# SinOncology/BreakID

Measured on AMD Instinct MI355X. Metric: M reads/s clustered+split-scanned, higher is better.
Workload: dtype int32/u8 (+f64 sd replay)

## Files before the change

### breakid_amd/csrc/sortemu.h

```cpp
#pragma once
#include "bk_common.h"
#include "prims.h"
#include <vector>
#include <atomic>

struct SortService
{
  DevBuf ctl, slots[2], seq[2], jobs, dbg, pos[2];
  uint32_t pos_cap[2] = {0, 0};
  uint32_t cap[2] = {0, 0};
  hipStream_t st[2] = {nullptr, nullptr}, quit_stream = nullptr, st_copy = nullptr;
  uint32_t *quit_host = nullptr;
  uint32_t *quit_dev = nullptr;
  uint32_t cap32 = 0;
  uint32_t quit_word = 0, starts = 0;
  size_t wide_lds = 0;
  bool running = false;
  std::atomic<uint32_t> next_slot{0};
  uint32_t stats[8] = {};
  void start(uint64_t n_bound, uint64_t max_group, hipStream_t after);
  bool narrow_running(double seconds) const;
  void stop();
  uint32_t new_slot() { return next_slot.fetch_add(1u); }
  ~SortService();
  SortService() = default;
  SortService(const SortService &) = delete;
  SortService &operator=(const SortService &) = delete;
};

struct SortEmuBufs
{
  SortService *svc = nullptr;
  uint32_t svc_slot = 0xFFFFFFFFu, svc_epoch = 0;
  DevBuf cnt, err, segs_a, segs_b, posL, posR, scan_tmp, heap_list, heap_scratch, scratch32, scratch32b, fin_list, lv_tile, lv_segbase, lv_tileseg, lv_bar, chk_key0, chk_cnt, chk_bad, rk_a, rk_b, heap_tickets;
  prims::RadixBufs radix;
  std::vector<uint32_t> *heavy = nullptr;
  bool heavy_all = false;
  bool fork_heaps = true;
  DevBuf tj_ctl, tj_jobs, tj_slots[2], tj_seq[2], tj_pos[2], tj_heavy, tj_trace;
  uint32_t tj_cap[2] = {0, 0}, tj_epoch = 0;
  bool tj_ready = false;
  uint64_t sorts[3] = {0, 0, 0};
  static constexpr int N_AUX = 5;
  hipStream_t aux[N_AUX] = {};
  hipEvent_t fork = nullptr, join[N_AUX] = {};
  SortEmuBufs() = default;
  SortEmuBufs(const SortEmuBufs &) = delete;
  SortEmuBufs &operator=(const SortEmuBufs &) = delete;
  ~SortEmuBufs()
  {
    for (int i = 0; i < N_AUX; ++i)
    {
      if (aux[i]) (void) hipStreamDestroy(aux[i]);
      if (join[i]) (void) hipEventDestroy(join[i]);
    }
    if (fork) (void) hipEventDestroy(fork);
  }
};

bool sort_tasks_on();

void std_sort_groups(uint32_t *key, uint32_t *idx, const uint32_t *gof, const uint64_t *goff, uint32_t ng, uint64_t n, SortEmuBufs &b, hipStream_t st);
```

### breakid_amd/csrc/sortemu.hip

```cpp
#include "bk_common.h"
#include "prims.h"
#include "sortemu.h"
#include <vector>
#include <mutex>
#include <algorithm>
#include <cstdio>
#include <chrono>
#include <thread>
#include <cstdlib>
#include <ctime>

namespace
{
inline double now_ms()
{
  timespec ts;
  clock_gettime(CLOCK_MONOTONIC, &ts);
  return ts.tv_sec * 1e3 + ts.tv_nsec * 1e-6;
}
typedef __attribute__((address_space(1))) uint32_t gu32_t;
__device__ __forceinline__ void st_through(uint32_t *p, uint32_t v) { __hip_atomic_store((gu32_t *) p, v, __ATOMIC_RELAXED, __HIP_MEMORY_SCOPE_AGENT); }
struct Seg
{
  uint32_t first, last;
  uint32_t pivot;
  int32_t depth;
  uint32_t cut;
  uint32_t cbase;
};

constexpr uint32_t FIN_MAX = 2048;
constexpr uint32_t HEAP_BIG_MIN = 4096;
constexpr uint32_t LV_TILE = 2048;
__device__ __forceinline__ void lv_mark_tiles(uint32_t *__restrict__ tile_seg, uint32_t s, uint32_t cbase, uint32_t size)
{
// ... 2230 lines not shown
__global__ __launch_bounds__(256) void k_chk_keys(const uint32_t *__restrict__ key, const uint32_t *__restrict__ idx, const uint32_t *__restrict__ key0, uint32_t n, uint32_t *__restrict__ bad)
{
  const uint32_t p = blockIdx.x * blockDim.x + threadIdx.x;
  if (p >= n) return;
  const uint32_t x = idx[p];
  if (x < n && key0[x] != key[p])
  {
    atomicAdd(&bad[4], 1u);
    atomicMin(&bad[5], p);
  }
}
static void sort_check(const char *phase, const uint32_t *key, const uint32_t *idx, const uint32_t *key0, uint32_t n, const uint64_t *goff, uint32_t ng, hipStream_t st, SortEmuBufs &b)
{
  uint32_t *c = b.chk_cnt.as<uint32_t>(n), *bd = b.chk_bad.as<uint32_t>(8);
  const uint32_t init[8] = {0, 0, 0xFFFFFFFFu, 0xFFFFFFFFu, 0, 0xFFFFFFFFu, 0, 0};
  HIP_CHECK(hipDeviceSynchronize());
  HIP_CHECK(hipMemset(c, 0, (size_t) n * 4));
  HIP_CHECK(hipMemcpy(bd, init, 32, hipMemcpyHostToDevice));
  hipLaunchKernelGGL(k_chk_count, dim3(cdiv(n, 256)), dim3(256), 0, st, idx, n, c, bd);
  hipLaunchKernelGGL(k_chk_keys, dim3(cdiv(n, 256)), dim3(256), 0, st, key, idx, key0, n, bd);
  uint32_t h[8];
  HIP_CHECK(hipMemcpyAsync(h, bd, 32, hipMemcpyDeviceToHost, st));
  HIP_CHECK(hipStreamSynchronize(st));
  if (h[0] || h[1] || h[4])
  {
    std::vector<uint64_t> go((size_t) ng + 1);
    HIP_CHECK(hipMemcpy(go.data(), goff, ((size_t) ng + 1) * 8, hipMemcpyDeviceToHost));
    auto grp = [&](uint32_t p) { return p == 0xFFFFFFFFu ? -1 : (int) (std::upper_bound(go.begin(), go.end(), (uint64_t) p) - go.begin()) - 1; };
    fprintf(stderr, "[sortemu] CHECK FAILED %s: %u payloads out of range (first at %u), %u duplicated payloads (first at position %u, group %d), %u elements whose key is not their own (first at %u, group %d); n=%u\n",
            phase, h[0], h[2], h[1], h[3], grp(h[3]), h[4], h[5], grp(h[5]), n);
  }
}

static SvcParams svc_params(SortService &S)
{
  SvcParams P;
  uint32_t *ctl = S.ctl.get<uint32_t>();
  for (int k = 0; k < 2; ++k)
  {
    P.q[k].head = ctl + 64 * k;
    P.q[k].tail = ctl + 64 * k + 32;
    P.q[k].slots = S.slots[k].get<SvcTask>();
    P.q[k].seq = S.seq[k].get<uint32_t>();
    P.q[k].mask = S.cap[k] - 1;
    P.q[k].release = 1u;
  }
  P.error = ctl + 128;
  P.stats = ctl + 160;
  P.jobs = S.jobs.get<SvcJob>();
  P.quit_d = ctl + 192;
  P.host = S.quit_dev;
  P.cap32 = S.cap32;
  P.quit_word = S.quit_word;
  P.dbg = S.dbg.get<uint32_t>();
  for (int k = 0; k < 2; ++k)
  {
    P.pos[k] = S.pos[k].get<uint32_t>();
    P.pos_cap[k] = S.pos_cap[k];
  }
  P.timeout_ticks = SVC_TIMEOUT_TICKS;
  return P;
}
void SortService::start(uint64_t n_bound, uint64_t max_group, hipStream_t after)
{
  if (running) return;
  quit_stream = after;
  int dev = 0, cus = 0;
  HIP_CHECK(hipGetDevice(&dev));
  HIP_CHECK(hipDeviceGetAttribute(&cus, hipDeviceAttributeMultiprocessorCount, dev));
  const int n_wide = std::min(1024, std::max(4, cus / 4));
  const int n_narrow = std::max(8, 2 * (cus - n_wide));
  if (!quit_host)
  {
    HIP_CHECK(hipHostMalloc(reinterpret_cast<void **>(&quit_host), SVC_H_WORDS * 4, hipHostMallocMapped));
    HIP_CHECK(hipHostGetDevicePointer(reinterpret_cast<void **>(&quit_dev), quit_host, 0));
    for (int k = 0; k < 2; ++k) HIP_CHECK(hipStreamCreateWithFlags(&st[k], hipStreamNonBlocking));
    HIP_CHECK(hipStreamCreateWithFlags(&st_copy, hipStreamNonBlocking));
    hipFuncAttributes fa;
    HIP_CHECK(hipFuncGetAttributes(&fa, reinterpret_cast<const void *>(k_sort_service<true>)));
    wide_lds = (size_t) ((160u * 1024u - (uint32_t) fa.sharedSizeBytes) & ~15u);
    cap32 = (uint32_t) (wide_lds / 4 - 3);
    if ((cap32 & 1u) == 0) --cap32;
    HIP_CHECK(hipFuncSetAttribute(reinterpret_cast<const void *>(k_sort_service<true>), hipFuncAttributeMaxDynamicSharedMemorySize, (int) wide_lds));
    HIP_CHECK(hipFuncSetAttribute(reinterpret_cast<const void *>(k_sort_service<false>), hipFuncAttributeMaxDynamicSharedMemorySize, (int) SVC_NARROW_LDS));
  }
  auto pow2 = [](uint64_t v) {
    uint32_t c = 1024;
    while (c < v && c < (1u << 30)) c <<= 1;
    return c;
  };
  cap[0] = pow2(n_bound / HEAP_BIG_MIN + 4096);
  cap[1] = pow2(n_bound / 16 + 4096);
  (void) ctl.as<uint32_t>(256);
  for (int k = 0; k < 2; ++k)
  {
    (void) slots[k].as<SvcTask>(cap[k]);
    (void) seq[k].as<uint32_t>(cap[k]);
  }
  (void) jobs.as<SvcJob>(SVC_MAX_JOBS);
  pos_cap[0] = (uint32_t) std::max<uint64_t>(max_group, SVC_WIDE_MIN) + 64;
  pos_cap[1] = SVC_WIDE_MIN + 64;
  (void) pos[0].as<uint32_t>(2ull * pos_cap[0] * (uint64_t) n_wide);
  (void) pos[1].as<uint32_t>(2ull * pos_cap[1] * (uint64_t) n_narrow);
  if (bk_debug("svc"))
  {
    (void) dbg.as<uint32_t>(12 * 8192 + 48);
    HIP_CHECK(hipMemsetAsync(dbg.p, 0, (12 * 8192 + 48) * 4, after));
  }
  __atomic_store_n(quit_host, 0u, __ATOMIC_SEQ_CST);
  quit_word = 0xC0DE0000u | (++starts & 0xFFFFu);
  for (uint32_t k = 1; k < SVC_H_WORDS; ++k) quit_host[k] = 0u;
  next_slot = 0;
  const SvcParams P = svc_params(*this);
  hipLaunchKernelGGL(k_svc_reset, dim3(cdiv(std::max(cap[0], cap[1]), 256)), dim3(256), 0, after, P);
  HIP_CHECK(hipStreamSynchronize(after));
// ... 17 lines not shown
}
bool SortService::narrow_running(double seconds) const
{
  const auto t0 = std::chrono::steady_clock::now();
  volatile const uint32_t *flag = quit_host + SVC_H_NARROW;
  while (*flag == 0u)
    if (std::chrono::duration<double>(std::chrono::steady_clock::now() - t0).count() > seconds) return false;
  return true;
}
void SortService::stop()
{
  if (!running) return;
  running = false;
  __atomic_store_n(quit_host, quit_word, __ATOMIC_SEQ_CST);
  (void) hipMemcpyAsync(ctl.get<uint32_t>() + 192, quit_host, 4, hipMemcpyHostToDevice, st_copy);
  hipLaunchKernelGGL(k_svc_quit, dim3(1), dim3(1), 0, quit_stream, ctl.get<uint32_t>() + 192, quit_word);
  HIP_CHECK(hipStreamSynchronize(st[0]));
  HIP_CHECK(hipStreamSynchronize(st[1]));
  uint32_t h[40] = {};
  HIP_CHECK(hipMemcpy(h, ctl.get<uint32_t>() + 128, sizeof h, hipMemcpyDeviceToHost));
  for (int k = 0; k < 8; ++k) stats[k] = h[32 + k];
  DeferredFrees::end();
  if (bk_debug("svc"))
  {
    uint32_t c[128] = {};
    SvcJob j0 = {};
    HIP_CHECK(hipMemcpy(c, ctl.get<uint32_t>(), sizeof c, hipMemcpyDeviceToHost));
    HIP_CHECK(hipMemcpy(&j0, jobs.get<SvcJob>(), sizeof j0, hipMemcpyDeviceToHost));
    if (dbg.p)
    {
      std::vector<uint32_t> d(12 * 8192 + 48);
      HIP_CHECK(hipMemcpy(d.data(), dbg.p, d.size() * 4, hipMemcpyDeviceToHost));
      {
        const uint32_t *ph = d.data() + 12 * 8192 + 32;
        const double lv = ph[7] ? (double) ph[7] : 1.0;
        fprintf(stderr, "[svc]   wide partition nodes: %u levels; per level: count pass %.2f us, place pass %.2f us, swaps + drain %.2f us, cut, release, pushes and the next pivot %.2f us\n", ph[7], ph[0] * 1e-2 / lv,
                ph[1] * 1e-2 / lv, ph[2] * 1e-2 / lv, ph[3] * 1e-2 / lv);
      }
      for (int kind = 0; kind < 2; ++kind)
      {
        fprintf(stderr, "[svc]   %s tasks by size (2^k ..):", kind ? "narrow heap" : "finisher");
        for (int k = 4; k < 13; ++k) fprintf(stderr, " %d:%u", k, d[12 * 8192 + 16 * kind + k]);
        fprintf(stderr, "\n");
      }
      for (int kind = 0; kind < 2; ++kind)
      {
        const uint32_t nw = kind == 0 ? stats[2] : stats[3];
        double sum[8] = {};
        uint32_t longest = 0;
        for (uint32_t w = 0; w < nw && w < 4096; ++w)
        {
          const uint32_t *a = d.data() + 4 * 8192 + 8 * (w + 4096 * kind);
          for (int k = 0; k < 7; ++k) sum[k] += a[k];
          longest = std::max(longest, a[7]);
        }
        fprintf(stderr, "[svc]   %s workgroups (%u): waiting %.2f ms; partition nodes %.0f in %.2f ms, finisher %.0f in %.2f ms, heaps %.0f in %.2f ms (sums over the workgroups); longest task %.3f ms\n", kind ? "narrow" : "wide", nw,
                sum[0] * 1e-5, sum[4], sum[1] * 1e-5, sum[5], sum[2] * 1e-5, sum[6], sum[3] * 1e-5, longest * 1e-5);
        std::map<uint32_t, int> hist;
        const uint32_t n = kind == 0 ? stats[2] : stats[3];
        for (uint32_t w = 0; w < n && w < 4096; ++w) hist[d[4 * (w + 4096 * kind)]]++;
        fprintf(stderr, "[svc]   %s workgroups by last state (1 polling, 5 took a task, 9 left):", kind ? "narrow" : "wide");
        for (auto &kv : hist) fprintf(stderr, " %u:%d", kv.first, kv.second);
        fprintf(stderr, "; first ones (state, polls, time of the last poll in 10 ns, how it left 6 error 7 quit 8 timeout):");
        for (uint32_t w = 0; w < 6 && w < n; ++w) fprintf(stderr, " [%u %u %u %u]", d[4 * (w + 4096 * kind)], d[4 * (w + 4096 * kind) + 1], d[4 * (w + 4096 * kind) + 2], d[4 * (w + 4096 * kind) + 3]);
        fprintf(stderr, "\n");
      }
    }
    uint32_t sq[4] = {};
    HIP_CHECK(hipMemcpy(sq, seq[1].get<uint32_t>(), sizeof sq, hipMemcpyDeviceToHost));
    fprintf(stderr, "[svc] tasks %u wide / %u narrow; workgroups started %u / %u, left on their own %u / %u, odd quit words read %u; error %u; wide queue head %u tail %u, narrow queue head %u tail %u (seq %u %u %u %u); job 0: remaining %u done %u heaps %u (longest %u)\n",
// ... 53 lines not shown
    {
      if (*err != 0u)
        throw bk_error(BK_ERR_HIP, "sort service: a task failed (error " + std::to_string(*err) + "; first failing task: code " + std::to_string(err[1]) + ", " + std::to_string(err[2]) + " " + std::to_string(err[3]) + " " + std::to_string(err[4]) + ")");
      if ((spins & 1023u) == 1023u)
      {
        if (std::chrono::duration<double>(std::chrono::steady_clock::now() - t0).count() > 20.0) throw bk_error(BK_ERR_HIP, "sort service: a job did not finish");
        std::this_thread::yield();
      }
      else
        __builtin_ia32_pause();
    }
  }
  if (bk_debug("svc"))
  {
    SvcJob j;
    HIP_CHECK(hipMemcpy(&j, S.jobs.get<SvcJob>() + b.svc_slot, sizeof j, hipMemcpyDeviceToHost));
    fprintf(stderr, "[svc] slot %u sort %u: %u elements in %u groups; partitions and finisher done after %.3f ms, job after %.3f ms; %u elements in heaps, the longest %u, the heap that ended last %u elements in %.3f ms\n", b.svc_slot,
            b.svc_epoch, n, ng, (double) (j.t_parts - j.t_submit) * 1e-5, (double) (j.t_done - j.t_submit) * 1e-5, j.n_heap, j.max_heap, (uint32_t) j.last_heap, (double) (j.last_heap >> 32) * 1e-5);
  }
  window_sorts(key, idx, gof, n, st);
}

static void std_sort_groups_tasks(uint32_t *key, uint32_t *idx, const uint32_t *gof, const uint64_t *goff, uint32_t ng, uint32_t n, SortEmuBufs &b, hipStream_t st, const uint32_t *key0)
{
  static size_t dyn_lds = 0;
  static uint32_t cap32 = 0;
  static std::once_flag once;
  std::call_once(once, [] {
    hipFuncAttributes fa;
    HIP_CHECK(hipFuncGetAttributes(&fa, reinterpret_cast<const void *>(k_sort_job)));
    dyn_lds = (size_t) ((160u * 1024u - (uint32_t) fa.sharedSizeBytes) & ~15u);
    cap32 = (uint32_t) (dyn_lds / 4 - 3);
    if ((cap32 & 1u) == 0) --cap32;
    if (dyn_lds < SJ_TEAMS * SJ_TEAM_LDS) throw bk_error(BK_ERR_HIP, "k_sort_job: the narrow teams do not fit the LDS");
    HIP_CHECK(hipFuncSetAttribute(reinterpret_cast<const void *>(k_sort_job), hipFuncAttributeMaxDynamicSharedMemorySize, (int) dyn_lds));
  });
  std::vector<uint64_t> go((size_t) ng + 1);
  HIP_CHECK(hipMemcpyAsync(go.data(), goff, go.size() * 8, hipMemcpyDeviceToHost, st));
  HIP_CHECK(hipStreamSynchronize(st));
  uint64_t max_group = 0;
  for (uint32_t g = 0; g < ng; ++g) max_group = std::max<uint64_t>(max_group, go[g + 1] - go[g]);
  const uint32_t n_wide = std::min<uint32_t>(SJ_MAX_WIDE, std::max<uint32_t>(1, cdiv(n, 1u << 16)));
  const uint32_t n_narrow = std::min<uint32_t>(SJ_MAX_NARROW, std::max<uint32_t>(1, cdiv(n, 1u << 16)));
  SjParams S = {};
  SvcParams &P = S.P;
  {
    auto pow2 = [](uint64_t v) {
      uint32_t c = 1024;
      while (c < v && c < (1u << 30)) c <<= 1;
      return c;
    };
    const uint32_t want[2] = {pow2((uint64_t) n / HEAP_BIG_MIN + 4096), pow2((uint64_t) n / 16 + 4096)};
    for (int k = 0; k < 2; ++k)
      if (want[k] > b.tj_cap[k])
      {
        b.tj_cap[k] = want[k];
        b.tj_ready = false;
      }
    uint32_t *ctl = b.tj_ctl.as<uint32_t>(SJ_C_WORDS);
    for (int k = 0; k < 2; ++k)
    {
      P.q[k].head = ctl + 64 * k;
      P.q[k].tail = ctl + 64 * k + 32;
      P.q[k].slots = b.tj_slots[k].as<SvcTask>(b.tj_cap[k]);
      P.q[k].seq = b.tj_seq[k].as<uint32_t>(b.tj_cap[k]);
      P.q[k].mask = b.tj_cap[k] - 1;
      P.q[k].release = 1u;
    }
    P.error = ctl + SJ_C_ERROR;
    P.stats = ctl + SJ_C_STATS;
    P.quit_d = ctl + SJ_C_QUIT;
    P.host = ctl + SJ_C_HOST;
    P.jobs = b.tj_jobs.as<SvcJob>(SVC_MAX_JOBS);
    P.cap32 = cap32;
    P.quit_word = 0u;
    P.timeout_ticks = SJ_TIMEOUT_TICKS;
    P.pos_cap[0] = (uint32_t) std::max<uint64_t>(max_group, SVC_WIDE_MIN) + 64;
    P.pos_cap[1] = SVC_WIDE_MIN + 64;
    P.pos[0] = b.tj_pos[0].as<uint32_t>(2ull * P.pos_cap[0] * n_wide);
    P.pos[1] = b.tj_pos[1].as<uint32_t>(2ull * P.pos_cap[1] * n_narrow * SJ_TEAMS);
    P.dbg = nullptr;
    S.n_wide = n_wide;
    S.live = ctl + SJ_C_LIVE;
    S.gof = gof;
    S.heavy_min = b.heavy_all ? FIN_MAX : HEAP_RANKED_MIN;
    if (b.heavy)
    {
      S.heavy = b.tj_heavy.as<uint32_t>(ng);
      HIP_CHECK(hipMemsetAsync(S.heavy, 0, (size_t) ng * 4, st));
    }
  }
  static const bool dbg = bk_debug("svc");
  if (dbg) S.trace = b.tj_trace.as<unsigned long long>(8);
  if (!b.tj_ready)
  {
    HIP_CHECK(hipMemsetAsync(b.tj_ctl.p, 0, SJ_C_WORDS * 4, st));
    hipLaunchKernelGGL(k_svc_reset, dim3(cdiv(std::max(b.tj_cap[0], b.tj_cap[1]), 256)), dim3(256), 0, st, P);
    b.tj_ready = true;
  }
  SvcJob d = {};
  d.key = key;
  d.idx = idx;
  d.hscratch = b.heap_scratch.as<hent>((uint64_t) n + HEAP_PAD);
  d.scratch32 = b.scratch32.as<uint32_t>((uint64_t) n + HEAP_PAD);
  d.scratch32b = b.scratch32b.as<uint32_t>((uint64_t) n + HEAP_PAD);
  d.rka = b.rk_a.as<unsigned long long>((uint64_t) n + HEAP_PAD);
  d.rkb = b.rk_b.as<unsigned long long>((uint64_t) n + HEAP_PAD);
  d.epoch = (b.tj_epoch++ % 0xFFFFFu) + 1u;
  const SvcJobLds J = {d.key, d.idx, nullptr, nullptr, d.hscratch, d.scratch32, d.scratch32b, d.rka, d.rkb, P.jobs, d.epoch << 8};
  hipLaunchKernelGGL(k_sort_job_submit, dim3(1), dim3(256), 0, st, S, d, goff, ng);
  hipLaunchKernelGGL(k_sort_job, dim3(n_wide + n_narrow), dim3(1024), dyn_lds, st, S, J);
  HIP_CHECK(hipGetLastError());
  ++b.sorts[1];
  if (key0) sort_check("after the task dispatch", key, idx, key0, n, goff, ng, st, b);
  window_sorts(key, idx, gof, n, st);
  uint32_t h[16] = {};
  HIP_CHECK(hipMemcpyAsync(h, P.error, 12 * 4, hipMemcpyDeviceToHost, st));
  std::vector<uint32_t> hv;
  if (S.heavy)
  {
    hv.resize(ng);
    HIP_CHECK(hipMemcpyAsync(hv.data(), S.heavy, (size_t) ng * 4, hipMemcpyDeviceToHost, st));
  }
  unsigned long long tr[8] = {};
  if (S.trace) HIP_CHECK(hipMemcpyAsync(tr, S.trace, 5 * 8, hipMemcpyDeviceToHost, st));
  SvcJob j = {};
  HIP_CHECK(hipMemcpyAsync(&j, P.jobs, sizeof j, hipMemcpyDeviceToHost, st));
  HIP_CHECK(hipStreamSynchronize(st));
  if (h[0] || j.remaining != 0u)
  {
    b.tj_ready = false;
    throw bk_error(h[0] & 2u ? BK_ERR_LIMIT : BK_ERR_HIP, "sort task dispatch: task error " + std::to_string(h[0]) + " (2 = ring overflow, 4 = no progress for 1 s, 8 = a cut outside its segment, 16 = a task in the wrong queue, 32 = a node beyond the position lists, 64 = the finisher), " + std::to_string(j.remaining) + " elements not final; first failing task: code " + std::to_string(h[8]) + ", " + std::to_string(h[9]) + " " + std::to_string(h[10]) + " " + std::to_string(h[11]));
  }
  if (S.heavy)
  {
    if (b.heavy->size() < ng) b.heavy->resize(ng, 0u);
    for (uint32_t g = 0; g < ng; ++g) (*b.heavy)[g] = std::max((*b.heavy)[g], hv[g]);
  }
  if (S.trace)
  {
    const double t0 = (double) tr[0];
    const uint32_t hm = (uint32_t) (tr[1] >> 40);
    const unsigned long long hs = tr[1] & 0xFFFFFFFFFFull, base = tr[0] & ~0xFFFFFFFFFFull;
    unsigned long long hstart = base | hs;
    if (hstart < tr[0]) hstart += 1ull << 40;
    fprintf(stderr, "[svc] task dispatch %u: %u elements in %u groups on %u wide + %u narrow workgroups; longest heap %u elements started %.3f ms after the dispatch and took %.3f ms; partitions and finisher done after %.3f ms, job after %.3f ms; %u elements in heaps, the longest %u\n",
            d.epoch, n, ng, n_wide, n_narrow, hm, hm ? ((double) hstart - t0) * 1e-5 : 0.0, hm ? (double) (tr[2] & 0xFFFFFFFFFFull) * 1e-5 : 0.0, tr[3] ? ((double) tr[3] - t0) * 1e-5 : 0.0, ((double) tr[4] - t0) * 1e-5, j.n_heap, j.max_heap);
  }
}

bool sort_tasks_on()
{
  static const bool on = !(getenv("BREAKID_SORT_TASKS") && atoi(getenv("BREAKID_SORT_TASKS")) == 0);
  return on;
}

void std_sort_groups(uint32_t *key, uint32_t *idx, const uint32_t *gof, const uint64_t *goff, uint32_t ng, uint64_t n64, SortEmuBufs &b, hipStream_t st)
{
  if (n64 == 0 || ng == 0) return;
  if (n64 > 0x7FFFFFF0ull) throw bk_error(BK_ERR_LIMIT, "std_sort_groups: more than 2^31 pairs");
  {
    static std::mutex flag_m;
    static bool flag_set[64] = {};
    int dev = 0;
    HIP_CHECK(hipGetDevice(&dev));
    std::lock_guard<std::mutex> l(flag_m);
    if (dev >= 0 && dev < 64 && !flag_set[dev])
    {
      const int nq = getenv("BK_HEAP_NO_Q") != nullptr;
      HIP_CHECK(hipMemcpyToSymbol(HIP_SYMBOL(g_heap_no_q), &nq, sizeof nq));
      const int nhy = nq;
      HIP_CHECK(hipMemcpyToSymbol(HIP_SYMBOL(g_heap_no_hybrid), &nhy, sizeof nhy));
      flag_set[dev] = true;
    }
  }
  const uint32_t n = (uint32_t) n64;
  if (b.svc && b.svc->running)
  {
    ++b.sorts[0];
    std_sort_groups_svc(key, idx, gof, goff, ng, n, b, st);
// ... 321 lines not shown
```

### breakid_amd/csrc/sortsvc.inc

```

constexpr uint32_t SVC_T_PART = 1, SVC_T_FIN = 2, SVC_T_HEAP = 3;
constexpr uint32_t SVC_WIDE_MIN = 16384;
constexpr uint32_t SVC_BIAS = 0x80000000u;
constexpr uint32_t SVC_MAX_JOBS = 64;
constexpr uint32_t SVC_H_QUIT = 0, SVC_H_ERROR = 1, SVC_H_NARROW = 8, SVC_H_STARTED = 16, SVC_H_DONE = SVC_H_STARTED + 1024, SVC_H_WORDS = SVC_H_DONE + SVC_MAX_JOBS;
constexpr uint32_t SVC_NARROW_LDS = 45056;
constexpr unsigned long long SVC_TIMEOUT_TICKS = 800000000ull;

struct SvcTask
{
  uint32_t type_job;
  uint32_t first, last;
  int32_t depth;
};
static_assert(sizeof(SvcTask) == 16, "two 8-byte halves");

struct SvcJob
{
  uint32_t *key, *idx, *posL, *posR;
  hent *hscratch;
  uint32_t *scratch32, *scratch32b;
  unsigned long long *rka, *rkb;
  uint32_t remaining;
  uint32_t done;
// ... 132 lines not shown
};

__device__ __forceinline__ uint32_t svc_pick_pivot(uint32_t first, uint32_t last, uint32_t *key, uint32_t *idx)
{
  const uint32_t a = first + 1, b = first + (last - first) / 2, c = last - 1;
  const uint32_t ka = key[a], kb = key[b], kc = key[c];
  uint32_t pick;
  if (ka < kb)
  {
    if (kb < kc) pick = b;
    else if (ka < kc) pick = c;
    else pick = a;
  }
  else if (ka < kc) pick = a;
  else if (kb < kc) pick = c;
  else pick = b;
  const uint32_t kf = key[first], kp = key[pick];
  const uint32_t xf = idx[first], xp = idx[pick];
  st_through(key + first, kp);
  st_through(key + pick, kf);
  st_through(idx + first, xp);
  st_through(idx + pick, xf);
  return kp;
}

template <uint32_t NT> struct SvcPartLds
{
  uint32_t first, last, pivot;
  int32_t depth;
  uint32_t cnt[2][NT / 64];
  uint32_t cut;
  int go_on;
};
template <uint32_t NT, bool WIDE, class T = WgTeam>
__device__ __forceinline__ void svc_part(const SvcParams &P, const SvcJobLds &J, SvcPartLds<NT> &S, const SvcTask t, uint32_t *pos, const uint32_t pos_cap, const T &team = T())
{
  constexpr uint32_t NW = NT / 64;
  const uint32_t tid = team.tid(), lane = tid & 63, w = tid >> 6;
  uint32_t *key = J.key, *idx = J.idx;
  const uint32_t job_tag = t.type_job >> 4;
  uint32_t retired = 0;
  if (tid == 0)
  {
    S.first = t.first;
    S.last = t.last;
    S.go_on = 1;
    if (t.depth == 0)
    {
      svc_push_heap(P, J.job, job_tag, t.first, t.last);
      S.go_on = 0;
    }
    else if (t.last - t.first > pos_cap + 1u)
    {
      atomicOr(P.error, 32u);
      S.go_on = 0;
    }
    else
    {
      S.pivot = svc_pick_pivot(t.first, t.last, key, idx);
      S.depth = t.depth - 1;
      S.cut = 0xFFFFFFFFu;
    }
  }
  team.sync();
  if (!S.go_on) return;
  unsigned long long tph = 0;
  uint32_t *phase = (P.dbg && WIDE) ? P.dbg + 12 * 8192 + 32 : nullptr;
  auto mark = [&](int k) {
    if (phase && tid == 0)
    {
      const unsigned long long now = wall_clock64();
      if (k >= 0) atomicAdd(phase + k, (uint32_t) (now - tph));
      tph = now;
    }
  };
  for (;;)
  {
    const uint32_t first = S.first, last = S.last, pivot = S.pivot;
    const int32_t depth = S.depth;
    mark(-1);
    if (phase && tid == 0) atomicAdd(phase + 7, 1u);
    const uint32_t lo = first + 1, total = last - lo;
    const uint32_t chunk = (((total + NW - 1) / NW) + 63u) & ~63u;
    const uint32_t wbeg = lo + min(total, w * chunk), wend = lo + min(total, (w + 1) * chunk);
    uint32_t cL = 0, cR = 0;
    {
      uint32_t p = wbeg + lane;
      for (; p + (TL_UNROLL - 1) * 64 < wend; p += TL_UNROLL * 64)
      {
        uint32_t k[TL_UNROLL];
#pragma unroll
        for (uint32_t u = 0; u < TL_UNROLL; ++u) k[u] = key[p + u * 64];
#pragma unroll
        for (uint32_t u = 0; u < TL_UNROLL; ++u)
        {
          cL += k[u] >= pivot ? 1u : 0u;
          cR += k[u] <= pivot ? 1u : 0u;
        }
      }
      for (; p < wend; p += 64)
      {
        const uint32_t k = key[p];
        cL += k >= pivot ? 1u : 0u;
        cR += k <= pivot ? 1u : 0u;
      }
    }
    for (int d = 32; d >= 1; d >>= 1)
    {
      cL += __shfl_xor(cL, d, 64);
      cR += __shfl_xor(cR, d, 64);
    }
    if (lane == 0)
    {
      S.cnt[0][w] = cL;
      S.cnt[1][w] = cR;
    }
    team.sync();
    mark(0);
    uint32_t runL = 0, runR = 0, nL = 0, nR = 0;
    for (uint32_t i = 0; i < NW; ++i)
    {
      const uint32_t a = S.cnt[0][i], b = S.cnt[1][i];
      if (i < w)
      {
        runL += a;
        runR += b;
      }
      nL += a;
      nR += b;
    }
    uint32_t *pL = pos, *pR = pos + pos_cap;
    {
      auto place = [&](uint32_t p, bool valid, uint32_t k) {
        const bool fL = valid && k >= pivot, fR = valid && k <= pivot;
        const unsigned long long mL = __ballot(fL), mR = __ballot(fR);
        const uint32_t bL = __builtin_amdgcn_mbcnt_hi((uint32_t) (mL >> 32), __builtin_amdgcn_mbcnt_lo((uint32_t) mL, 0u));
        const uint32_t bR = __builtin_amdgcn_mbcnt_hi((uint32_t) (mR >> 32), __builtin_amdgcn_mbcnt_lo((uint32_t) mR, 0u));
        if (fL) pL[runL + bL] = p;
        if (fR) pR[runR + bR] = p;
        runL += (uint32_t) __popcll(mL);
        runR += (uint32_t) __popcll(mR);
      };
      uint32_t p0 = wbeg;
      for (; p0 + TL_UNROLL * 64 <= wend; p0 += TL_UNROLL * 64)
      {
        uint32_t k[TL_UNROLL];
#pragma unroll
        for (uint32_t u = 0; u < TL_UNROLL; ++u) k[u] = key[p0 + u * 64 + lane];
#pragma unroll
        for (uint32_t u = 0; u < TL_UNROLL; ++u) place(p0 + u * 64 + lane, true, k[u]);
      }
      for (; p0 < wend; p0 += 64)
      {
        const uint32_t p = p0 + lane;
        const bool valid = p < wend;
        place(p, valid, valid ? key[p] : 0u);
      }
    }
    team.sync();
    mark(1);
    const uint32_t mm = nL < nR ? nL : nR;
    constexpr uint32_t SW = 4;
    for (uint32_t j0 = tid; j0 <= mm; j0 += SW * NT)
    {
      uint32_t lj[SW], rj[SW];
      bool sw[SW];
#pragma unroll
      for (uint32_t u = 0; u < SW; ++u)
      {
        const uint32_t j = j0 + u * NT;
        lj[u] = j < nL ? pL[j] : 0xFFFFFFFFu;
        rj[u] = j < nR ? pR[nR - 1 - j] : first;
      }
      uint32_t k1[SW], k2[SW], x1[SW], x2[SW];
#pragma unroll
      for (uint32_t u = 0; u < SW; ++u)
      {
        const uint32_t j = j0 + u * NT;
        sw[u] = j <= mm && (j < nL) && (j < nR) && (lj[u] < rj[u]);
        if (sw[u])
        {
          k1[u] = key[lj[u]];
          k2[u] = key[rj[u]];
          x1[u] = idx[lj[u]];
          x2[u] = idx[rj[u]];
        }
      }
#pragma unroll
      for (uint32_t u = 0; u < SW; ++u)
        if (sw[u])
        {
          st_through(key + lj[u], k2[u]);
          st_through(key + rj[u], k1[u]);
          st_through(idx + lj[u], x2[u]);
          st_through(idx + rj[u], x1[u]);
        }
#pragma unroll
      for (uint32_t u = 0; u < SW; ++u)
      {
        const uint32_t j = j0 + u * NT;
        if (j > mm || sw[u]) continue;
        const uint32_t ljj = lj[u];
        bool prev_cont = false;
        uint32_t rprev = 0;
        if (j > 0)
        {
          const uint32_t lp = pL[j - 1];
          rprev = pR[nR - j];
          prev_cont = lp < rprev;
        }
        if (j == 0)
          S.cut = ljj;
        else if (prev_cont)
          S.cut = ljj < rprev ? ljj : rprev;
      }
      if (!sw[SW - 1]) break;
    }
    svc_drain_barrier(team);
    mark(2);
    const uint32_t cut = S.cut;
    team.sync();
    if (cut == 0xFFFFFFFFu || cut <= first || cut > last)
    {
      if (tid == 0) SVC_FAIL(P, 8u, first, last, cut);
      return;
    }
    if (tid == 0)
    {
      const uint32_t a0 = first, a1 = cut, b0 = cut, b1 = last;
      const uint32_t sa = a1 - a0, sb = b1 - b0;
      const bool big_is_a = sa >= sb;
      const uint32_t g0 = big_is_a ? a0 : b0, g1 = big_is_a ? a1 : b1, h0 = big_is_a ? b0 : a0, h1 = big_is_a ? b1 : a1;
      const uint32_t sg = g1 - g0, sh = h1 - h0;
      const bool carry = sg > FIN_MAX && (!WIDE || sg > SVC_WIDE_MIN);
      const bool push_g = sg > 16 && !carry, push_h = sh > 16;
      retired += (sg <= 16 ? sg : 0u) + (sh <= 16 ? sh : 0u);
      const bool carry_heap = carry && depth == 0;
      if (push_g || push_h || carry_heap)
      {
        team.count_pushes((push_h ? 1u : 0u) + (push_g ? 1u : 0u));
        if (P.q[0].release & 1u) svc_release();
        if (push_h)
        {
          if (sh <= FIN_MAX)
            svc_push(P.q[1], SvcTask{svc_tag(SVC_T_FIN, job_tag), h0, h1, depth}, P.error);
          else
            svc_push_part(P, job_tag, h0, h1, depth);
        }
        if (push_g)
        {
// ... 6 lines not shown
      }
      if (carry && !carry_heap)
      {
        S.first = g0;
        S.last = g1;
        S.pivot = svc_pick_pivot(g0, g1, key, idx);
        S.depth = depth - 1;
        S.cut = 0xFFFFFFFFu;
        S.go_on = 1;
      }
      else
        S.go_on = 0;
    }
    svc_drain_barrier(team);
    mark(3);
    if (!S.go_on) break;
  }
  if (tid == 0 && retired) svc_retire(P, J.job, job_tag, retired);
}

constexpr uint32_t F2_HB = 256;
constexpr uint32_t F2_QCAP = 256;
constexpr uint32_t F2_EXT = 16;
struct Fin2Lds
{
  hent ent[FIN_MAX];
  uint16_t posL[FIN_MAX + 2], posR[FIN_MAX + 2];
  unsigned long long q[F2_QCAP];
  hent hbuf[4][F2_HB + 4];
  uint2 ext[F2_EXT];
  uint32_t q_head, q_tail, pending, n_ext, ext_elems, bad;
};
static_assert(sizeof(Fin2Lds) <= SVC_NARROW_LDS, "narrow workgroup LDS");
static_assert(FIN_MAX / F2_HB + 1 <= F2_EXT && FIN_MAX / 17 + 8 <= F2_QCAP, "fin2 lists");

__device__ __forceinline__ void f2_wsync()
{
  __builtin_amdgcn_fence(__ATOMIC_ACQ_REL, "wavefront");
  __builtin_amdgcn_wave_barrier();
}
__device__ __forceinline__ void f2_push(Fin2Lds &L, uint32_t first, uint32_t last, int32_t depth)
{
  const uint32_t slot = atomicAdd(&L.q_tail, 1u);
  if (slot >= F2_QCAP)
  {
    L.bad = 1u;
    return;
  }
  __hip_atomic_store(&L.q[slot], (unsigned long long) first | ((unsigned long long) last << 16) | ((unsigned long long) (uint32_t) (depth + 1) << 32), __ATOMIC_RELEASE, __HIP_MEMORY_SCOPE_WORKGROUP);
}
__device__ __forceinline__ uint32_t f2_partition(Fin2Lds &L, const uint32_t first, const uint32_t last, const uint32_t lane)
{
  hent *ent = L.ent;
  const uint32_t a = first + 1, b = first + (last - first) / 2, c = last - 1;
  const hent ea = ent[a], eb = ent[b], ec = ent[c];
  const uint32_t ka = hkey(ea), kb = hkey(eb), kc = hkey(ec);
  uint32_t pick;
  if (ka < kb)
  {
    if (kb < kc) pick = b;
    else if (ka < kc) pick = c;
    else pick = a;
  }
  else if (ka < kc) pick = a;
  else if (kb < kc) pick = c;
  else pick = b;
// ... 253 lines not shown
#pragma unroll
          for (int k = 0; k < 9; ++k) v[k] = svc_read(src + k);
          s_job.key = (uint32_t *) v[0];
          s_job.idx = (uint32_t *) v[1];
          s_job.posL = (uint32_t *) v[2];
          s_job.posR = (uint32_t *) v[3];
          s_job.hscratch = (hent *) v[4];
          s_job.scratch32 = (uint32_t *) v[5];
          s_job.scratch32b = (uint32_t *) v[6];
          s_job.rka = (unsigned long long *) v[7];
          s_job.rkb = (unsigned long long *) v[8];
          s_job.job = job;
          s_job.tag = tag;
        }
        s_task = t;
      }
      s_state = st;
      if (dbg) SVC_ST(dbg, st == 1 ? 5u : 9u);
      t_task = wall_clock64();
      acc[0] += (uint32_t) (t_task - t_poll);
      if (dbg && st != 1)
      {
        uint32_t *a = P.dbg + 4 * 8192 + 8 * (blockIdx.x + (WIDE ? 0u : 4096u));
        for (int k = 0; k < 8; ++k) SVC_ST(a + k, acc[k]);
      }
    }
    __syncthreads();
    if (s_state != 1) return;
    const SvcTask t = s_task;
    const uint32_t type = t.type_job & 15u;
    if (P.dbg && tid == 0 && !WIDE && type != SVC_T_PART)
      atomicAdd(P.dbg + 12 * 8192 + (type == SVC_T_HEAP ? 16 : 0) + (31 - __clz((int) (t.last - t.first))), 1u);
    if (type == SVC_T_PART)
      svc_part<NT, WIDE>(P, s_job, s_part, t, P.pos[WIDE ? 0 : 1] + 2ull * P.pos_cap[WIDE ? 0 : 1] * blockIdx.x, P.pos_cap[WIDE ? 0 : 1]);
    else if (type == SVC_T_HEAP)
    {
      if (WIDE)
        heap_big_body(t.first, t.last, s_job.key, s_job.idx, s_job.hscratch, s_job.scratch32, s_job.scratch32b, s_job.rka, s_job.rkb, reinterpret_cast<hent *>(pool), P.cap32, NT);
      else
        heap_small_body(t.first, t.last, s_job.key, s_job.idx, reinterpret_cast<hent *>(pool), NT);
      svc_drain_barrier();
      if (tid == 0) svc_retire(P, s_job.job, t.type_job >> 4, t.last - t.first);
    }
    else if (type == SVC_T_FIN && !WIDE)
    {
      Fin2Lds &L = *reinterpret_cast<Fin2Lds *>(pool);
      fin2_body(L, t.first, t.last, t.depth, s_job.key, s_job.idx);
      svc_drain_barrier();
      if (tid == 0)
      {
        if (L.bad) SVC_FAIL(P, 64u, t.first, t.last, L.bad | (L.q_tail << 8) | (L.n_ext << 20));
        const uint32_t nh = L.n_ext < F2_EXT ? L.n_ext : F2_EXT;
        if (nh && (P.q[0].release & 1u)) svc_release();
        for (uint32_t k = 0; k < nh; ++k) svc_push_heap(P, s_job.job, t.type_job >> 4, L.ext[k].x, L.ext[k].y);
        svc_retire(P, s_job.job, t.type_job >> 4, (t.last - t.first) - L.ext_elems);
      }
    }
    else if (tid == 0)
      atomicOr(P.error, 16u);
    if (tid == 0)
    {
      t_last = wall_clock64();
      atomicAdd(P.stats + (WIDE ? 0 : 1), 1u);
      if (P.dbg)
      {
        if (type == SVC_T_HEAP)
          s_job.job->last_heap = ((unsigned long long) (t_last - t_task) << 32) | (t.last - t.first);
// ... 117 lines not shown
        if ((polls & 7u) == 0)
        {
          if (svc_read(P.error) != 0u || svc_read(&job->remaining) == 0u)
          {
            st = 2;
            break;
          }
          if (svc_read(S.live) == 0u)
          {
            st = svc_take(q, ticket, t) ? 1 : 2;
            break;
          }
          if (wall_clock64() - t_last > P.timeout_ticks)
          {
            SVC_FAIL(P, 4u, WIDE ? 1u : 0u, svc_read(&job->remaining), svc_read(S.live));
            st = 2;
            break;
          }
        }
        for (uint32_t k = 0; k < nap; ++k) __builtin_amdgcn_s_sleep(32);
        if (nap < 4) ++nap;
      }
      if (st == 1) svc_acquire();
      s_task = t;
      s_state = st;
      t_task = wall_clock64();
    }
    team.sync();
    if (s_state != 1) return;
    const SvcTask t = s_task;
    const uint32_t type = t.type_job & 15u, job_tag = t.type_job >> 4;
    if (type == SVC_T_PART)
    {
      svc_part<NT, WIDE, T>(P, J, s_part, t, pos, P.pos_cap[WIDE ? 0 : 1], team);
      if (tid == 0)
      {
        asm volatile("s_waitcnt vmcnt(0)" ::: "memory");
        atomicSub(S.live, 1u);
      }
    }
    else if (type == SVC_T_HEAP)
    {
      const uint32_t m = t.last - t.first;
      if (WIDE)
        heap_big_body(t.first, t.last, J.key, J.idx, J.hscratch, J.scratch32, J.scratch32b, J.rka, J.rkb, reinterpret_cast<hent *>(pool), P.cap32, NT);
      else
        heap_small_body<T>(t.first, t.last, J.key, J.idx, reinterpret_cast<hent *>(pool), NT, team);
      svc_drain_barrier(team);
      if (tid == 0)
      {
        if (S.heavy && m > S.heavy_min) atomicMax(S.heavy + S.gof[t.first], m);
        if (S.trace)
        {
          const unsigned long long now = wall_clock64();
          atomicMax(S.trace + 1, ((unsigned long long) m << 40) | (t_task & 0xFFFFFFFFFFull));
          atomicMax(S.trace + 2, ((unsigned long long) m << 40) | ((now - t_task) & 0xFFFFFFFFFFull));
        }
        svc_retire(P, job, job_tag, m);
      }
    }
    else if (type == SVC_T_FIN && !WIDE)
    {
      Fin2Lds &L = *reinterpret_cast<Fin2Lds *>(pool);
      fin2_body<T>(L, t.first, t.last, t.depth, J.key, J.idx, team);
      svc_drain_barrier(team);
      if (tid == 0)
      {
// ... 103 lines not shown
```

Baseline: 11850.

## Partition via LDS row ballot masks and compact swap lists instead of global position passes

```diff
diff --git a/breakid_amd/csrc/partlevels.h b/breakid_amd/csrc/partlevels.h
--- /dev/null
+++ b/breakid_amd/csrc/partlevels.h
@@ -0,0 +1,57 @@
+#pragma once
+#include <cstdint>
+
+#if defined(__HIPCC__)
+#define PL_HD __host__ __device__ __forceinline__
+#else
+#define PL_HD inline
+#endif
+
+constexpr uint32_t PL_NONE = 0xFFFFFFFFu;
+
+PL_HD uint32_t pl_list_len(uint32_t n_kind, uint32_t mm) { return n_kind < mm + 1u ? n_kind : mm + 1u; }
+
+PL_HD bool pl_fits_rows(uint32_t first, uint32_t last, uint32_t rows_cap) { return last - first - 1u <= rows_cap * 64u; }
+PL_HD bool pl_fits_lists(uint32_t nL, uint32_t nR, uint32_t list_cap) { return (nL < nR ? nL : nR) + 1u <= list_cap; }
+
+PL_HD uint32_t pl_chunk(uint32_t total, uint32_t nw) { return (((total + nw - 1u) / nw) + 63u) & ~63u; }
+
+PL_HD uint32_t pl_nth_bit(unsigned long long m, uint32_t rank)
+{
+  for (; rank; --rank) m &= m - 1ull;
+  return (uint32_t) __builtin_ctzll(m);
+}
+template <class Prefix> PL_HD uint32_t pl_row_of(const Prefix &excl, uint32_t rows, uint32_t rank)
+{
+  uint32_t lo = 0, hi = rows;
+  while (hi - lo > 1u)
+  {
+    const uint32_t mid = lo + (hi - lo) / 2u;
+    if (excl(mid) <= rank) lo = mid; else hi = mid;
+  }
+  return lo;
+}
+PL_HD uint32_t pl_from_right(uint32_t n, uint32_t j) { return n - 1u - j; }
+
+template <class List> PL_HD void pl_expand_left(unsigned long long m, uint32_t E, uint32_t len, uint32_t row_pos, List &&list)
+{
+  for (uint32_t i = E; m != 0ull && i < len; ++i, m &= m - 1ull) list(i, row_pos + (uint32_t) __builtin_ctzll(m));
+}
+template <class List> PL_HD void pl_expand_right(unsigned long long m, uint32_t E, uint32_t n, uint32_t len, uint32_t row_pos, List &&list)
+{
+  uint32_t j = n - E - (uint32_t) __builtin_popcountll(m);
+  for (; m != 0ull && j < len; ++j)
+  {
+    const uint32_t b = 63u - (uint32_t) __builtin_clzll(m);
+    list(j, row_pos + b);
+    m &= ~(1ull << b);
+  }
+}
+
+PL_HD bool pl_swapped(uint32_t j, uint32_t nL, uint32_t nR, uint32_t lj, uint32_t rj) { return j < nL && j < nR && lj < rj; }
+PL_HD uint32_t pl_cut_at(uint32_t j, uint32_t lj, uint32_t lprev, uint32_t rprev)
+{
+  if (j == 0) return lj;
+  if (lprev < rprev) return lj < rprev ? lj : rprev;
+  return PL_NONE;
+}
diff --git a/breakid_amd/csrc/sortemu.h b/breakid_amd/csrc/sortemu.h
--- a/breakid_amd/csrc/sortemu.h
+++ b/breakid_amd/csrc/sortemu.h
@@ -37,7 +37,7 @@
   std::vector<uint32_t> *heavy = nullptr;
   bool heavy_all = false;
   bool fork_heaps = true;
-  DevBuf tj_ctl, tj_jobs, tj_slots[2], tj_seq[2], tj_pos[2], tj_heavy, tj_trace;
+  DevBuf tj_ctl, tj_jobs, tj_slots[2], tj_seq[2], tj_pos[2], tj_heavy, tj_trace, tj_dbg;
   uint32_t tj_cap[2] = {0, 0}, tj_epoch = 0;
   bool tj_ready = false;
   uint64_t sorts[3] = {0, 0, 0};
diff --git a/breakid_amd/csrc/sortemu.hip b/breakid_amd/csrc/sortemu.hip
--- a/breakid_amd/csrc/sortemu.hip
+++ b/breakid_amd/csrc/sortemu.hip
@@ -1,6 +1,7 @@
 #include "bk_common.h"
 #include "prims.h"
 #include "sortemu.h"
+#include "partlevels.h"
 #include <vector>
 #include <mutex>
 #include <algorithm>
@@ -2297,6 +2298,18 @@
   }
 }
 
+static uint32_t svc_release_bits()
+{
+  static const bool lists = !(getenv("BREAKID_PART_LISTS") && atoi(getenv("BREAKID_PART_LISTS")) == 0);
+  return 1u | (lists ? 0u : 4u);
+}
+
+static void svc_print_levels(const uint32_t *ph)
+{
+  const double lv = ph[7] ? (double) ph[7] : 1.0;
+  fprintf(stderr, "[svc]   wide partition nodes: %u levels, %u of them by the count + place passes; per level: classify (or count pass) %.2f us, expand (or place pass) %.2f us, swaps + drain %.2f us, cut, release, pushes and the next pivot %.2f us\n",
+          ph[7], ph[8], ph[0] * 1e-2 / lv, ph[1] * 1e-2 / lv, ph[2] * 1e-2 / lv, ph[3] * 1e-2 / lv);
+}
 static SvcParams svc_params(SortService &S)
 {
   SvcParams P;
@@ -2308,7 +2321,7 @@
     P.q[k].slots = S.slots[k].get<SvcTask>();
     P.q[k].seq = S.seq[k].get<uint32_t>();
     P.q[k].mask = S.cap[k] - 1;
-    P.q[k].release = 1u;
+    P.q[k].release = svc_release_bits();
   }
   P.error = ctl + 128;
   P.stats = ctl + 160;
@@ -2346,6 +2359,7 @@
     wide_lds = (size_t) ((160u * 1024u - (uint32_t) fa.sharedSizeBytes) & ~15u);
     cap32 = (uint32_t) (wide_lds / 4 - 3);
     if ((cap32 & 1u) == 0) --cap32;
+    if (wide_lds < PL_WIDE_LDS) throw bk_error(BK_ERR_HIP, "k_sort_service: the row masks of a wide partition node do not fit the LDS");
     HIP_CHECK(hipFuncSetAttribute(reinterpret_cast<const void *>(k_sort_service<true>), hipFuncAttributeMaxDynamicSharedMemorySize, (int) wide_lds));
     HIP_CHECK(hipFuncSetAttribute(reinterpret_cast<const void *>(k_sort_service<false>), hipFuncAttributeMaxDynamicSharedMemorySize, (int) SVC_NARROW_LDS));
   }
@@ -2429,10 +2443,7 @@
       std::vector<uint32_t> d(12 * 8192 + 48);
       HIP_CHECK(hipMemcpy(d.data(), dbg.p, d.size() * 4, hipMemcpyDeviceToHost));
       {
-        const uint32_t *ph = d.data() + 12 * 8192 + 32;
-        const double lv = ph[7] ? (double) ph[7] : 1.0;
-        fprintf(stderr, "[svc]   wide partition nodes: %u levels; per level: count pass %.2f us, place pass %.2f us, swaps + drain %.2f us, cut, release, pushes and the next pivot %.2f us\n", ph[7], ph[0] * 1e-2 / lv,
-                ph[1] * 1e-2 / lv, ph[2] * 1e-2 / lv, ph[3] * 1e-2 / lv);
+        svc_print_levels(d.data() + 12 * 8192 + 32);
       }
       for (int kind = 0; kind < 2; ++kind)
       {
@@ -2552,6 +2563,7 @@
     dyn_lds = (size_t) ((160u * 1024u - (uint32_t) fa.sharedSizeBytes) & ~15u);
     cap32 = (uint32_t) (dyn_lds / 4 - 3);
     if ((cap32 & 1u) == 0) --cap32;
+    if (dyn_lds < PL_WIDE_LDS) throw bk_error(BK_ERR_HIP, "k_sort_job: the row masks of a wide partition node do not fit the LDS");
     if (dyn_lds < SJ_TEAMS * SJ_TEAM_LDS) throw bk_error(BK_ERR_HIP, "k_sort_job: the narrow teams do not fit the LDS");
     HIP_CHECK(hipFuncSetAttribute(reinterpret_cast<const void *>(k_sort_job), hipFuncAttributeMaxDynamicSharedMemorySize, (int) dyn_lds));
   });
@@ -2585,7 +2597,7 @@
       P.q[k].slots = b.tj_slots[k].as<SvcTask>(b.tj_cap[k]);
       P.q[k].seq = b.tj_seq[k].as<uint32_t>(b.tj_cap[k]);
       P.q[k].mask = b.tj_cap[k] - 1;
-      P.q[k].release = 1u;
+      P.q[k].release = svc_release_bits();
     }
     P.error = ctl + SJ_C_ERROR;
     P.stats = ctl + SJ_C_STATS;
@@ -2611,7 +2623,12 @@
     }
   }
   static const bool dbg = bk_debug("svc");
-  if (dbg) S.trace = b.tj_trace.as<unsigned long long>(8);
+  if (dbg)
+  {
+    S.trace = b.tj_trace.as<unsigned long long>(8);
+    P.dbg = b.tj_dbg.as<uint32_t>(12 * 8192 + 48);
+    HIP_CHECK(hipMemsetAsync(P.dbg + 12 * 8192 + 32, 0, 16 * 4, st));
+  }
   if (!b.tj_ready)
   {
     HIP_CHECK(hipMemsetAsync(b.tj_ctl.p, 0, SJ_C_WORDS * 4, st));
@@ -2644,6 +2661,8 @@
   }
   unsigned long long tr[8] = {};
   if (S.trace) HIP_CHECK(hipMemcpyAsync(tr, S.trace, 5 * 8, hipMemcpyDeviceToHost, st));
+  uint32_t ph[16] = {};
+  if (P.dbg) HIP_CHECK(hipMemcpyAsync(ph, P.dbg + 12 * 8192 + 32, 16 * 4, hipMemcpyDeviceToHost, st));
   SvcJob j = {};
   HIP_CHECK(hipMemcpyAsync(&j, P.jobs, sizeof j, hipMemcpyDeviceToHost, st));
   HIP_CHECK(hipStreamSynchronize(st));
@@ -2666,6 +2685,7 @@
     if (hstart < tr[0]) hstart += 1ull << 40;
     fprintf(stderr, "[svc] task dispatch %u: %u elements in %u groups on %u wide + %u narrow workgroups; longest heap %u elements started %.3f ms after the dispatch and took %.3f ms; partitions and finisher done after %.3f ms, job after %.3f ms; %u elements in heaps, the longest %u\n",
             d.epoch, n, ng, n_wide, n_narrow, hm, hm ? ((double) hstart - t0) * 1e-5 : 0.0, hm ? (double) (tr[2] & 0xFFFFFFFFFFull) * 1e-5 : 0.0, tr[3] ? ((double) tr[3] - t0) * 1e-5 : 0.0, ((double) tr[4] - t0) * 1e-5, j.n_heap, j.max_heap);
+    svc_print_levels(ph);
   }
 }
 
diff --git a/breakid_amd/csrc/sortsvc.inc b/breakid_amd/csrc/sortsvc.inc
--- a/breakid_amd/csrc/sortsvc.inc
+++ b/breakid_amd/csrc/sortsvc.inc
@@ -188,10 +188,23 @@
   uint32_t cut;
   int go_on;
 };
+template <bool WIDE> struct PartRows
+{
+  static constexpr uint32_t ROWS = WIDE ? 4096u : 256u, CAP = WIDE ? 8192u : 2048u;
+  unsigned long long mL[ROWS], mR[ROWS];
+  uint16_t eL[ROWS], eR[ROWS];
+  uint32_t listL[CAP], listR[CAP];
+};
+constexpr size_t PL_WIDE_LDS = 160u * 1024u - 4096u;
+static_assert(sizeof(PartRows<true>) <= PL_WIDE_LDS, "wide workgroup LDS");
+static_assert(PartRows<false>::ROWS * 64u >= SVC_WIDE_MIN && (PartRows<true>::ROWS * 64u / 16u + 64u) < 65536u, "row prefixes are 16-bit");
+
 template <uint32_t NT, bool WIDE, class T = WgTeam>
-__device__ __forceinline__ void svc_part(const SvcParams &P, const SvcJobLds &J, SvcPartLds<NT> &S, const SvcTask t, uint32_t *pos, const uint32_t pos_cap, const T &team = T())
+__device__ __forceinline__ void svc_part(const SvcParams &P, const SvcJobLds &J, SvcPartLds<NT> &S, const SvcTask t, uint32_t *pos, const uint32_t pos_cap, unsigned char *pool, const T &team = T())
 {
   constexpr uint32_t NW = NT / 64;
+  PartRows<WIDE> &R = *reinterpret_cast<PartRows<WIDE> *>(pool);
+  const bool two_pass = (P.q[0].release & 4u) != 0u;
   const uint32_t tid = team.tid(), lane = tid & 63, w = tid >> 6;
   uint32_t *key = J.key, *idx = J.idx;
   const uint32_t job_tag = t.type_job >> 4;
@@ -237,9 +250,43 @@
     mark(-1);
     if (phase && tid == 0) atomicAdd(phase + 7, 1u);
     const uint32_t lo = first + 1, total = last - lo;
-    const uint32_t chunk = (((total + NW - 1) / NW) + 63u) & ~63u;
+    const uint32_t chunk = pl_chunk(total, NW);
     const uint32_t wbeg = lo + min(total, w * chunk), wend = lo + min(total, (w + 1) * chunk);
     uint32_t cL = 0, cR = 0;
+    const bool rows = !two_pass && pl_fits_rows(first, last, PartRows<WIDE>::ROWS);
+    if (rows)
+    {
+      uint32_t r = (wbeg - lo) >> 6;
+      auto classify = [&](bool valid, uint32_t k) {
+        const unsigned long long mL = __ballot(valid && k >= pivot), mR = __ballot(valid && k <= pivot);
+        if (lane == 0)
+        {
+          R.mL[r] = mL;
+          R.mR[r] = mR;
+          R.eL[r] = (uint16_t) cL;
+          R.eR[r] = (uint16_t) cR;
+        }
+        cL += (uint32_t) __popcll(mL);
+        cR += (uint32_t) __popcll(mR);
+        ++r;
+      };
+      uint32_t p0 = wbeg;
+      for (; p0 + TL_UNROLL * 64 <= wend; p0 += TL_UNROLL * 64)
+      {
+        uint32_t k[TL_UNROLL];
+#pragma unroll
+        for (uint32_t u = 0; u < TL_UNROLL; ++u) k[u] = key[p0 + u * 64 + lane];
+#pragma unroll
+        for (uint32_t u = 0; u < TL_UNROLL; ++u) classify(true, k[u]);
+      }
+      for (; p0 < wend; p0 += 64)
+      {
+        const uint32_t p = p0 + lane;
+        const bool valid = p < wend;
+        classify(valid, valid ? key[p] : 0u);
+      }
+    }
+    else
     {
       uint32_t p = wbeg + lane;
       for (; p + (TL_UNROLL - 1) * 64 < wend; p += TL_UNROLL * 64)
@@ -260,11 +307,11 @@
         cL += k >= pivot ? 1u : 0u;
         cR += k <= pivot ? 1u : 0u;
       }
-    }
-    for (int d = 32; d >= 1; d >>= 1)
-    {
-      cL += __shfl_xor(cL, d, 64);
-      cR += __shfl_xor(cR, d, 64);
+      for (int d = 32; d >= 1; d >>= 1)
+      {
+        cL += __shfl_xor(cL, d, 64);
+        cR += __shfl_xor(cR, d, 64);
+      }
     }
     if (lane == 0)
     {
@@ -285,7 +332,24 @@
       nL += a;
       nR += b;
     }
+    const uint32_t mm = nL < nR ? nL : nR;
+    const bool lists = rows && pl_fits_lists(nL, nR, PartRows<WIDE>::CAP);
+    if (phase && tid == 0 && !lists) atomicAdd(phase + 8, 1u);
     uint32_t *pL = pos, *pR = pos + pos_cap;
+    if (lists)
+    {
+      const uint32_t lenL = pl_list_len(nL, mm), lenR = pl_list_len(nR, mm);
+      const uint32_t r0 = (wbeg - lo) >> 6, r1 = wbeg < wend ? (wend - lo + 63u) >> 6 : r0;
+      for (uint32_t r = r0 + lane; r < r1; r += 64)
+      {
+        const uint32_t row_pos = lo + (r << 6);
+        const uint32_t eL = runL + R.eL[r], eR = runR + R.eR[r];
+        if (eL < lenL) pl_expand_left(R.mL[r], eL, lenL, row_pos, [&](uint32_t i, uint32_t p) { R.listL[i] = p; });
+        const unsigned long long mR = R.mR[r];
+        if (nR - eR - (uint32_t) __popcll(mR) < lenR) pl_expand_right(mR, eR, nR, lenR, row_pos, [&](uint32_t j, uint32_t p) { R.listR[j] = p; });
+      }
+    }
+    else
     {
       auto place = [&](uint32_t p, bool valid, uint32_t k) {
         const bool fL = valid && k >= pivot, fR = valid && k <= pivot;
@@ -315,7 +379,7 @@
     }
     team.sync();
     mark(1);
-    const uint32_t mm = nL < nR ? nL : nR;
+    auto swaps = [&](auto l, auto r) {
     constexpr uint32_t SW = 4;
     for (uint32_t j0 = tid; j0 <= mm; j0 += SW * NT)
     {
@@ -325,15 +389,15 @@
       for (uint32_t u = 0; u < SW; ++u)
       {
         const uint32_t j = j0 + u * NT;
-        lj[u] = j < nL ? pL[j] : 0xFFFFFFFFu;
-        rj[u] = j < nR ? pR[nR - 1 - j] : first;
+        lj[u] = j < nL && j <= mm ? l(j) : PL_NONE;
+        rj[u] = j < nR && j <= mm ? r(j) : first;
       }
       uint32_t k1[SW], k2[SW], x1[SW], x2[SW];
 #pragma unroll
       for (uint32_t u = 0; u < SW; ++u)
       {
         const uint32_t j = j0 + u * NT;
-        sw[u] = j <= mm && (j < nL) && (j < nR) && (lj[u] < rj[u]);
+        sw[u] = j <= mm && pl_swapped(j, nL, nR, lj[u], rj[u]);
         if (sw[u])
         {
           k1[u] = key[lj[u]];
@@ -356,22 +420,16 @@
       {
         const uint32_t j = j0 + u * NT;
         if (j > mm || sw[u]) continue;
-        const uint32_t ljj = lj[u];
-        bool prev_cont = false;
-        uint32_t rprev = 0;
-        if (j > 0)
-        {
-          const uint32_t lp = pL[j - 1];
-          rprev = pR[nR - j];
-          prev_cont = lp < rprev;
-        }
-        if (j == 0)
-          S.cut = ljj;
-        else if (prev_cont)
-          S.cut = ljj < rprev ? ljj : rprev;
+        const uint32_t c = pl_cut_at(j, lj[u], j ? l(j - 1) : 0u, j ? r(j - 1) : 0u);
+        if (c != PL_NONE || j == 0) S.cut = c;
       }
       if (!sw[SW - 1]) break;
     }
+    };
+    if (lists)
+      swaps([&](uint32_t j) { return R.listL[j]; }, [&](uint32_t j) { return R.listR[j]; });
+    else
+      swaps([&](uint32_t j) { return pL[j]; }, [&](uint32_t j) { return pR[pl_from_right(nR, j)]; });
     svc_drain_barrier(team);
     mark(2);
     const uint32_t cut = S.cut;
@@ -444,6 +502,7 @@
   uint32_t q_head, q_tail, pending, n_ext, ext_elems, bad;
 };
 static_assert(sizeof(Fin2Lds) <= SVC_NARROW_LDS, "narrow workgroup LDS");
+static_assert(sizeof(PartRows<false>) <= sizeof(Fin2Lds), "a narrow team partitions in the LDS its finisher has");
 static_assert(FIN_MAX / F2_HB + 1 <= F2_EXT && FIN_MAX / 17 + 8 <= F2_QCAP, "fin2 lists");
 
 __device__ __forceinline__ void f2_wsync()
@@ -763,7 +822,7 @@
     if (P.dbg && tid == 0 && !WIDE && type != SVC_T_PART)
       atomicAdd(P.dbg + 12 * 8192 + (type == SVC_T_HEAP ? 16 : 0) + (31 - __clz((int) (t.last - t.first))), 1u);
     if (type == SVC_T_PART)
-      svc_part<NT, WIDE>(P, s_job, s_part, t, P.pos[WIDE ? 0 : 1] + 2ull * P.pos_cap[WIDE ? 0 : 1] * blockIdx.x, P.pos_cap[WIDE ? 0 : 1]);
+      svc_part<NT, WIDE>(P, s_job, s_part, t, P.pos[WIDE ? 0 : 1] + 2ull * P.pos_cap[WIDE ? 0 : 1] * blockIdx.x, P.pos_cap[WIDE ? 0 : 1], pool);
     else if (type == SVC_T_HEAP)
     {
       if (WIDE)
@@ -947,7 +1006,7 @@
     const uint32_t type = t.type_job & 15u, job_tag = t.type_job >> 4;
     if (type == SVC_T_PART)
     {
-      svc_part<NT, WIDE, T>(P, J, s_part, t, pos, P.pos_cap[WIDE ? 0 : 1], team);
+      svc_part<NT, WIDE, T>(P, J, s_part, t, pos, P.pos_cap[WIDE ? 0 : 1], pool, team);
       if (tid == 0)
       {
         asm volatile("s_waitcnt vmcnt(0)" ::: "memory");
```

After: 11560. -2.5%, worse.
